# fgnt/pb_chime5

Hardware: AMD Instinct MI355X
Metric: utterance-seconds enhanced/sec/GPU (24ch, 20 EM iters) (higher is better)
Workload: dtype f64

## Files before the change

### pb_chime5_amd/csrc/wpe.hip

```cpp
#include <algorithm>
#include <cmath>
#include <cstdlib>

#include "gss_internal.h"
#include <type_traits>
#include "dense_wave.h"

typedef double v4d __attribute__((ext_vector_type(4)));

namespace {

constexpr int POW_FRAMES = 256;
__global__ __launch_bounds__(POW_FRAMES) void wpe_power_kernel(const cplx *__restrict__ X,
                                                               int64_t T, int D, int psd_context,
                                                               double *__restrict__ raw,
                                                               double *__restrict__ w) {
    extern __shared__ __attribute__((aligned(16))) char smem[];
    double *ps = reinterpret_cast<double *>(smem);
    __shared__ double red[POW_FRAMES / 64];
    const int f = blockIdx.x, tid = threadIdx.x;
    const cplx *Xf = X + (int64_t)f * T * D;
    double *wout = w + (int64_t)f * T;
    double *wf = psd_context > 0 ? raw + (int64_t)f * T : wout;
    const int DP = D + 1;
// ... 553 lines not shown
    if (threadIdx.x == 0 && blockIdx.x < 8192) {
        g_corr_trace[blockIdx.x * 6 + 0] = xcd;
        g_corr_trace[blockIdx.x * 6 + 1] = wall_clock64();
        g_corr_trace[blockIdx.x * 6 + 2] = clock64();
    }
#endif
    int live = 0;
    if (threadIdx.x == 0) {
        ring[0] = corr_fetch(counters, F, xcd, live, cq);
        ring[1] = ring[0] < 0 ? -1 : corr_fetch(counters, F, xcd, live, cq);
        ring[2] = -1;
    }
    __syncthreads();

    const uint32_t lane16 = lane * 16;
    auto issue = [&](int fq, int64_t t0, int bq) {
        const __amdgpu_buffer_rsrc_t rsrc_y = __builtin_amdgcn_make_buffer_rsrc(
            const_cast<cplx *>(Y + (int64_t)fq * T * D), 0, (int)(T * D * 16), 0x00020000);
        cplx *Sb = S0 + bq * win;
        const int64_t g0 = (t0 - c) * (int64_t)D;
        if (g0 >= 0 && g0 + win <= T * (int64_t)D) {
            for (int p = wave; p < pieces; p += NW)
                __builtin_amdgcn_raw_ptr_buffer_load_lds(rsrc_y, (lds_void_ptr)(Sb + p * 64), 16,
                                                         lane16, (int)((g0 + p * 64) * 16), 0, 0);
        } else {
            for (int p = wave; p < pieces; p += NW) {
                const int64_t gp = g0 + p * 64;
                const uint32_t voff = (uint32_t)((gp + lane) * 16);
                if (gp >= 0) {
                    __builtin_amdgcn_raw_ptr_buffer_load_lds(rsrc_y, (lds_void_ptr)(Sb + p * 64),
                                                             16, voff, 0, 0, 0);
                } else if (gp + lane < 0) {
                    Sb[p * 64 + lane] = c_make(0.0, 0.0);
                } else {
                    __builtin_amdgcn_raw_ptr_buffer_load_lds(rsrc_y, (lds_void_ptr)(Sb + p * 64),
                                                             16, voff, 0, 0, 0);
                }
            }
        }
        if (wave == NW - 1 && lane < CORR_KT / 2) {
            const __amdgpu_buffer_rsrc_t rsrc_w = __builtin_amdgcn_make_buffer_rsrc(
                const_cast<double *>(w + (int64_t)fq * T), 0, (int)(T * 8), 0x00020000);
            __builtin_amdgcn_raw_ptr_buffer_load_lds(rsrc_w, (lds_void_ptr)(w0 + bq * CORR_KT), 16,
                                                     lane16, (int)(t0 * 8), 0, 0);
        }
    };

    int item = __builtin_amdgcn_readfirstlane(ring[0]);
    if (item < 0) return;
    int b = 0;
    issue(item >> 12, 0, 0);
    __syncthreads();
    for (int k = 0; item >= 0; ++k) {
        const int next = __builtin_amdgcn_readfirstlane(ring[(k + 1) % 3]);
        int fetched = -1;
        if (threadIdx.x == 0 && next >= 0) fetched = corr_fetch(counters, F, xcd, live, cq);
        const int f = item >> 12, grp = item & 4095;
        const int tile_id = grp * NW + wave;
        const bool active = tile_id < ntiles;
        const CorrTile tl = tiles[active ? tile_id : 0];
        const int mask = __builtin_amdgcn_readfirstlane(active ? tl.mask : 1);
        int *ring_slot = &ring[(k + 2) % 3];
#define CORR_CASE(M)                                                                              \
    case M:                                                                                       \
        corr_item_dma<M, NW, BLOCKED>(T, D, n, c, win, S0, w0, tl, active, f, next < 0 ? -1 : next >> 12, \
                                 b, issue, ring_slot, fetched, R, P);                             \
        break
#define CORR_CASE_RG(RG)                                                                          \
    case 15 + 16 * RG:                                                                            \
        if constexpr (!BLOCKED)                                                                   \
            corr_item_dma<15 + 16 * RG, NW, false>(T, D, n, c, win, S0, w0, tl, active, f,        \
                                                   next < 0 ? -1 : next >> 12, b, issue,          \
                                                   ring_slot, fetched, R, P);                     \
        break
        switch (BLOCKED ? mask & 15 : mask) {
            CORR_CASE(1);
            CORR_CASE(3);
            CORR_CASE(5);
            CORR_CASE(11);
            CORR_CASE_RG(1);
            CORR_CASE_RG(2);
            CORR_CASE_RG(3);
            default:
                corr_item_dma<15, NW, BLOCKED>(T, D, n, c, win, S0, w0, tl, active, f,
                                          next < 0 ? -1 : next >> 12, b, issue, ring_slot, fetched,
                                          R, P);
        }
#undef CORR_CASE
#undef CORR_CASE_RG
        item = next;
#ifdef GSS_CORR_TRACE
        if (threadIdx.x == 0 && blockIdx.x < 8192) {
            g_corr_trace[blockIdx.x * 6 + 3] = wall_clock64();
            g_corr_trace[blockIdx.x * 6 + 4] = clock64();
            g_corr_trace[blockIdx.x * 6 + 5] = k + 1;
        }
#endif
    }
}

#ifndef GSS_UPD_PREFETCH
#define GSS_UPD_PREFETCH 1
#endif
constexpr int CH_NB = 48;
constexpr int UD_LD = CH_NB + 1;

constexpr size_t DIAG_LDS = sizeof(cplx) * 2 * UD_LD + sizeof(double) * CH_NB;

__device__ inline void chol_diag_block(cplx *A, int n, int j0, cplx *Ud, double *dinv,
                                       int32_t *zero_pivots) {
    const int tid = threadIdx.x, tx = tid & 15, ty = tid >> 4;
    const int nb = min(CH_NB, n - j0);
    cplx reg[3][3];
#pragma unroll
    for (int a = 0; a < 3; ++a)
#pragma unroll
        for (int b = 0; b < 3; ++b) {
            const int i = ty + 16 * a, k = tx + 16 * b;
            reg[a][b] = (k >= i && k < nb) ? A[(int64_t)(j0 + i) * n + j0 + k] : c_make(0.0, 0.0);
        }
    if (!chol_inverse_sweep<16, 3, false, true>(reg, nb, Ud, UD_LD, dinv, tx, ty)) {
        if (tid < nb && dinv[tid] == 0.0) atomicAdd(zero_pivots, 1);
    }
#pragma unroll
    for (int a = 0; a < 3; ++a) {
        const int i = ty + 16 * a;
        const double di = i < nb ? dinv[i] : 0.0;
#pragma unroll
        for (int b = 0; b < 3; ++b) {
            const int k = tx + 16 * b;
            if (b < a || i >= nb || k >= nb) continue;
            const cplx raw = reg[a][b];
            A[(int64_t)(j0 + i) * n + j0 + k] =
                k == i ? c_make(di > 0.0 ? sqrt(raw.x) : 0.0, 0.0) : c_scale(raw, di);
        }
    }
}

__global__ __launch_bounds__(256) void chol_diag_kernel(cplx *__restrict__ R, int n, int j0,
                                                        int32_t *__restrict__ zero_pivots) {
    __shared__ __attribute__((aligned(16))) char smem[DIAG_LDS];
    cplx *Ud = reinterpret_cast<cplx *>(smem);
    double *dinv = reinterpret_cast<double *>(Ud + 2 * UD_LD);
    chol_diag_block(R + (int64_t)blockIdx.x * n * n, n, j0, Ud, dinv, zero_pivots);
}

constexpr int UDP_SIZE = 16 * (CH_NB + 1) + 16 * (CH_NB - 16 + 1) + 16 * (CH_NB - 32 + 1);
__device__ __forceinline__ int udp_off(int row, int col) {
    const int b = row >> 4;
    const int base = b == 0 ? 0 : b == 1 ? 16 * (CH_NB + 1) : 16 * (CH_NB + 1) + 16 * (CH_NB - 16 + 1);
    return base + (row & 15) * (CH_NB - 16 * b + 1) + col - 16 * b;
}

__device__ inline void chol_panel_tile(cplx *A, cplx *Z, int n, int D, int j0, int nb, int ct,
                                       const cplx *Ud, const double *dinv, int lane) {
    const int ntrail = n - j0 - nb;
    const int li = lane & 15, lk = lane >> 4;
    const int nct_a = (ntrail + 15) / 16;
    cplx *base;
    int64_t stride;
    int ncols;
    if (ct < nct_a) {
        base = A + (int64_t)j0 * n + j0 + nb + 16 * ct;
        stride = n;
        ncols = min(16, ntrail - 16 * ct);
    } else {
        base = Z + (int64_t)j0 * D + 16 * (ct - nct_a);
        stride = D;
        ncols = min(16, D - 16 * (ct - nct_a));
    }
    cplx bv[CH_NB / 4];
#pragma unroll
    for (int ks = 0; ks < CH_NB / 4; ++ks) {
        const int row = 4 * ks + lk;
        bv[ks] = (row < nb && li < ncols) ? base[row * stride + li] : c_make(0.0, 0.0);
    }
    v4d xre[3], xim[3];
#pragma unroll
    for (int it = 0; it < 3; ++it) {
        v4d tre, tim;
#pragma unroll
        for (int r = 0; r < 4; ++r) {
            tre[r] = bv[4 * it + r].x;
            tim[r] = bv[4 * it + r].y;
        }
        const int i = 16 * it + li;
#pragma unroll
        for (int jt = 0; jt < it; ++jt)
#pragma unroll
            for (int ks = 0; ks < 4; ++ks) {
                const int k = 16 * jt + 4 * ks + lk;
                const cplx u = Ud[udp_off(k, i)];
                tre = __builtin_amdgcn_mfma_f64_16x16x4f64(-u.x, xre[jt][ks], tre, 0, 0, 0);
                tim = __builtin_amdgcn_mfma_f64_16x16x4f64(-u.x, xim[jt][ks], tim, 0, 0, 0);
                tre = __builtin_amdgcn_mfma_f64_16x16x4f64(-u.y, xim[jt][ks], tre, 0, 0, 0);
                tim = __builtin_amdgcn_mfma_f64_16x16x4f64(u.y, xre[jt][ks], tim, 0, 0, 0);
            }
        xre[it] = (v4d){0.0, 0.0, 0.0, 0.0};
        xim[it] = (v4d){0.0, 0.0, 0.0, 0.0};
#pragma unroll
        for (int ks = 0; ks < 4; ++ks) {
            const int k = 16 * it + 4 * ks + lk;
            cplx w = Ud[udp_off(i, k)];
            if (k == i) w = c_make(i < nb ? dinv[i] : 0.0, 0.0);
            if (k > i) w = c_make(0.0, 0.0);
            xre[it] = __builtin_amdgcn_mfma_f64_16x16x4f64(w.x, tre[ks], xre[it], 0, 0, 0);
            xim[it] = __builtin_amdgcn_mfma_f64_16x16x4f64(w.x, tim[ks], xim[it], 0, 0, 0);
            xre[it] = __builtin_amdgcn_mfma_f64_16x16x4f64(-w.y, tim[ks], xre[it], 0, 0, 0);
            xim[it] = __builtin_amdgcn_mfma_f64_16x16x4f64(w.y, tre[ks], xim[it], 0, 0, 0);
        }
    }
#pragma unroll
    for (int it = 0; it < 3; ++it)
#pragma unroll
        for (int r = 0; r < 4; ++r) {
            const int row = 16 * it + lk + 4 * r;
            if (row < nb && li < ncols) base[row * stride + li] = c_make(xre[it][r], xim[it][r]);
        }
}

__device__ inline void chol_stage_diag(const cplx *A, int n, int j0, int nb, cplx *Ud, double *dinv) {
    const int tid = threadIdx.x;
    constexpr int WL = CH_NB * CH_NB / 256;
    static_assert(WL * 256 == CH_NB * CH_NB, "block size");
    cplx wv[WL];
#pragma unroll
    for (int s = 0; s < WL; ++s) {
        const int idx = tid + 256 * s;
        const int i = idx / CH_NB, k = idx - i * CH_NB;
        wv[s] = c_make(0.0, 0.0);
        if (i < nb && k < nb && k >= (i & ~15)) wv[s] = A[(int64_t)(j0 + i) * n + j0 + k];
    }
#pragma unroll
    for (int s = 0; s < WL; ++s) {
        const int idx = tid + 256 * s;
        const int i = idx / CH_NB, k = idx - i * CH_NB;
        if (k >= (i & ~15)) Ud[udp_off(i, k)] = wv[s];
        if (k == i) dinv[i] = wv[s].x > 0.0 ? 1.0 / wv[s].x : 0.0;
    }
}

__global__ __launch_bounds__(256) void chol_trsm_kernel(cplx *__restrict__ R,
                                                        cplx *__restrict__ P, int F, int n,
                                                        int D, int j0) {
    extern __shared__ __attribute__((aligned(16))) char smem[];
    cplx *Ud = reinterpret_cast<cplx *>(smem);
    double *dinv = reinterpret_cast<double *>(Ud + UDP_SIZE);
    const int tid = threadIdx.x;
    const int nb = min(CH_NB, n - j0);
    const int ntrail = n - j0 - nb;
    const int npanel = (ntrail + 15) / 16 + (D + 15) / 16;
    int f, grp;
    if (!xcd_group_map((npanel + 3) / 4, F, f, grp)) return;
    cplx *A = R + (int64_t)f * n * n;
    cplx *Z = P + (int64_t)f * n * D;
    chol_stage_diag(A, n, j0, nb, Ud, dinv);
    __syncthreads();
    const int ct = grp * 4 + (tid >> 6);
    if (ct < npanel) chol_panel_tile(A, Z, n, D, j0, nb, ct, Ud, dinv, tid & 63);
}

struct UpdTile {
    int row_off, col_off, is_p, pad;
};

template <int TM, int TN, bool PREFETCH>
__device__ inline void chol_update_tile(cplx *A, cplx *Z, int n, int D, int j0, int nb,
                                        const UpdTile tl, int lane) {
    const int li = lane & 15, lk = lane >> 4;
    const cplx *panel = A + (int64_t)j0 * n;
    const cplx *zpanel = Z + (int64_t)j0 * D;
    const int ncols = tl.is_p ? D : n;

    auto load_ops = [&](int ks, cplx (&a)[TM], cplx (&b)[TN]) {
        const int kk = 4 * ks + lk;
        const bool kv = kk < nb;
#pragma unroll
        for (int m = 0; m < TM; ++m) {
            const int ri = tl.row_off + 16 * m + li;
            a[m] = (kv && ri < n) ? panel[(int64_t)kk * n + ri] : c_make(0.0, 0.0);
        }
#pragma unroll
        for (int m = 0; m < TN; ++m) {
            const int ci = tl.col_off + 16 * m + li;
            b[m] = c_make(0.0, 0.0);
            if (kv && ci < ncols)
                b[m] = tl.is_p ? zpanel[(int64_t)kk * D + ci] : panel[(int64_t)kk * n + ci];
        }
    };

    const int ksteps = (nb + 3) / 4;
    cplx a_cur[TM], b_cur[TN];
    load_ops(0, a_cur, b_cur);

    cplx cv[TM][TN][4];
#pragma unroll
    for (int a = 0; a < TM; ++a)
#pragma unroll
        for (int b = 0; b < TN; ++b)
#pragma unroll
            for (int reg = 0; reg < 4; ++reg) {
                const int r = tl.row_off + 16 * a + lk + 4 * reg;
                const int c = tl.col_off + 16 * b + li;
                cv[a][b][reg] = c_make(0.0, 0.0);
                if (r < n && c < ncols) cv[a][b][reg] = tl.is_p ? Z[(int64_t)r * D + c] : A[(int64_t)r * n + c];
            }
    v4d t1[TM][TN], t2[TM][TN], t3[TM][TN];
#pragma unroll
    for (int a = 0; a < TM; ++a)
#pragma unroll
        for (int b = 0; b < TN; ++b) {
            t1[a][b] = (v4d){0.0, 0.0, 0.0, 0.0};
            t2[a][b] = (v4d){0.0, 0.0, 0.0, 0.0};
            t3[a][b] = (v4d){0.0, 0.0, 0.0, 0.0};
        }
    constexpr int PD = GSS_UPD_PREFETCH;
    cplx a_ring[PD][TM], b_ring[PD][TN];
#pragma unroll
    for (int p = 0; p < PD; ++p)
        if (PREFETCH && p + 1 < ksteps) load_ops(p + 1, a_ring[p], b_ring[p]);
    for (int ks = 0; ks < ksteps; ++ks) {
        cplx a_new[TM], b_new[TN];
        if (PREFETCH) {
            if (ks + PD + 1 < ksteps) load_ops(ks + PD + 1, a_new, b_new);
        } else if (ks > 0) {
            load_ops(ks, a_cur, b_cur);
        }
        double as[TM], bd[TN];
#pragma unroll
        for (int m = 0; m < TM; ++m) as[m] = a_cur[m].x + a_cur[m].y;
#pragma unroll
        for (int m = 0; m < TN; ++m) bd[m] = b_cur[m].x - b_cur[m].y;
#pragma unroll
        for (int a = 0; a < TM; ++a)
#pragma unroll
            for (int b = 0; b < TN; ++b) {
                t1[a][b] = __builtin_amdgcn_mfma_f64_16x16x4f64(a_cur[a].x, b_cur[b].x, t1[a][b], 0, 0, 0);
                t2[a][b] = __builtin_amdgcn_mfma_f64_16x16x4f64(a_cur[a].y, b_cur[b].y, t2[a][b], 0, 0, 0);
                t3[a][b] = __builtin_amdgcn_mfma_f64_16x16x4f64(as[a], bd[b], t3[a][b], 0, 0, 0);
            }
        if (PREFETCH) {
#pragma unroll
            for (int m = 0; m < TM; ++m) {
                a_cur[m] = a_ring[0][m];
#pragma unroll
                for (int p = 0; p + 1 < PD; ++p) a_ring[p][m] = a_ring[p + 1][m];
                a_ring[PD - 1][m] = a_new[m];
            }
#pragma unroll
            for (int m = 0; m < TN; ++m) {
                b_cur[m] = b_ring[0][m];
#pragma unroll
                for (int p = 0; p + 1 < PD; ++p) b_ring[p][m] = b_ring[p + 1][m];
                b_ring[PD - 1][m] = b_new[m];
            }
        }
    }
#pragma unroll
    for (int a = 0; a < TM; ++a)
#pragma unroll
        for (int b = 0; b < TN; ++b)
#pragma unroll
            for (int reg = 0; reg < 4; ++reg) {
                const int r = tl.row_off + 16 * a + lk + 4 * reg;
                const int c = tl.col_off + 16 * b + li;
                if (r < n && c < ncols) {
                    const cplx v = c_make(cv[a][b][reg].x - (t1[a][b][reg] + t2[a][b][reg]),
                                          cv[a][b][reg].y - ((t1[a][b][reg] - t2[a][b][reg]) - t3[a][b][reg]));
                    if (tl.is_p) Z[(int64_t)r * D + c] = v;
                    else A[(int64_t)r * n + c] = v;
                }
            }
}

constexpr int UPD_WAVES = 4;

template <int TM, int TN, bool PREFETCH>
__global__ __launch_bounds__(64 * UPD_WAVES) void chol_update_kernel(cplx *__restrict__ R,
                                                          cplx *__restrict__ P, int F, int n,
                                                          int D, int j0, int nb,
                                                          const UpdTile *__restrict__ tiles,
                                                          int ntiles, int ndiag, int j0_next,
                                                          int32_t *__restrict__ zero_pivots) {
    __shared__ __attribute__((aligned(16))) char smem[DIAG_LDS];
    const int F8 = ndiag > 0 ? (F + 7) / 8 * 8 : 0;
    const bool diag_group = (int)blockIdx.x < F8;
    int f, grp;
    if (diag_group) {
        f = blockIdx.x;
        grp = 0;
        if (f >= F) return;
    } else {
        const int L = blockIdx.x - F8, nsub = (ntiles - ndiag + UPD_WAVES - 1) / UPD_WAVES;
        const int sg = L / (8 * nsub), rem = L - sg * 8 * nsub;
        grp = rem >> 3;
        f = sg * 8 + (rem & 7);
        if (f >= F) return;
    }
    const int wave = __builtin_amdgcn_readfirstlane(threadIdx.x >> 6), lane = threadIdx.x & 63;
    cplx *A = R + (int64_t)f * n * n, *Z = P + (int64_t)f * n * D;
    if (diag_group) {
        __builtin_amdgcn_s_setprio(3);
        for (int t = wave; t < ndiag; t += UPD_WAVES)
            chol_update_tile<TM, TN, PREFETCH>(A, Z, n, D, j0, nb, tiles[t], lane);
        __syncthreads();
        if (wave >= 4) return;
        cplx *Ud = reinterpret_cast<cplx *>(smem);
        double *dinv = reinterpret_cast<double *>(Ud + 2 * UD_LD);
        chol_diag_block(A, n, j0_next, Ud, dinv, zero_pivots);
        return;
    }
    const int tile_id = ndiag + grp * UPD_WAVES + wave;
    if (tile_id >= ntiles) return;
    chol_update_tile<TM, TN, PREFETCH>(A, Z, n, D, j0, nb, tiles[tile_id], lane);
}

constexpr int BS_LD = 33;
constexpr int BS_OPS = 6 * 4 * 64;

__device__ inline void chol_backsolve_body(const cplx *A, cplx *Z, int n, int D, cplx *S,
                                           cplx *OP) {
    const int wave = __builtin_amdgcn_readfirstlane(threadIdx.x >> 6), lane = threadIdx.x & 63;
    const int li = lane & 15, lk = lane >> 4;
    const int nblk = (n + CH_NB - 1) / CH_NB;
    const int a = wave;
    for (int c0 = 0; c0 < D; c0 += 32) {
        for (int J = nblk - 1; J >= 0; --J) {
            const int j0 = J * CH_NB, nb = min(CH_NB, n - j0);
            if (a == 3) {
                const cplx *Ad = A + (int64_t)j0 * n + j0;
                auto fetch = [&](int row, int col) {
                    const bool ok = row < nb && col < nb;
                    const cplx v = Ad[(int64_t)(ok ? row : 0) * n + (ok ? col : 0)];
                    return c_make(ok ? v.x : 0.0, ok ? v.y : 0.0);
                };
                cplx wop[3][4], uop[3][4];
                double dg[3];
#pragma unroll
                for (int it = 0; it < 3; ++it) {
#pragma unroll
                    for (int ks = 0; ks < 4; ++ks) wop[it][ks] = fetch(16 * it + 4 * ks + lk, 16 * it + li);
                    dg[it] = fetch(16 * it + li, 16 * it + li).x;
                }
#pragma unroll
                for (int ks = 0; ks < 4; ++ks) {
                    uop[0][ks] = fetch(16 + li, 32 + 4 * ks + lk);
                    uop[1][ks] = fetch(li, 16 + 4 * ks + lk);
                    uop[2][ks] = fetch(li, 32 + 4 * ks + lk);
                }
#pragma unroll
                for (int it = 0; it < 3; ++it) {
                    const double ndinv = dg[it] > 0.0 ? -1.0 / dg[it] : 0.0;
#pragma unroll
                    for (int ks = 0; ks < 4; ++ks) {
                        const int k = 4 * ks + lk;
                        const cplx w = wop[it][ks];
                        OP[(it * 4 + ks) * 64 + lane] =
                            c_make(k == li ? ndinv : (k < li ? 0.0 : -w.x), k <= li ? 0.0 : -w.y);
                        OP[((3 + it) * 4 + ks) * 64 + lane] = uop[it][ks];
                    }
                }
            } else {
                v4d acc_re[2], acc_im[2];
#pragma unroll
                for (int b = 0; b < 2; ++b)
#pragma unroll
                    for (int reg = 0; reg < 4; ++reg) {
                        const int rl = 16 * a + lk + 4 * reg, col = c0 + 16 * b + li;
                        cplx v = c_make(0.0, 0.0);
                        if (rl < nb && col < D) v = Z[(int64_t)(j0 + rl) * D + col];
                        acc_re[b][reg] = v.x;
                        acc_im[b][reg] = v.y;
                    }
                const int kbeg = j0 + nb;
                const int ksteps = (n - kbeg + 3) / 4;
                const int arow = 16 * a + li;
                auto load_ops = [&](int ks, cplx &u, cplx (&g)[2]) {
                    const int kk = kbeg + 4 * ks + lk;
                    const bool kv = kk < n;
                    u = (kv && arow < nb) ? A[(int64_t)(j0 + arow) * n + kk] : c_make(0.0, 0.0);
#pragma unroll
                    for (int b = 0; b < 2; ++b) {
                        const int col = c0 + 16 * b + li;
                        g[b] = (kv && col < D) ? Z[(int64_t)kk * D + col] : c_make(0.0, 0.0);
                    }
                };
                constexpr int PD = 6;
                cplx u_r[PD], g_r[PD][2];
#pragma unroll
                for (int p = 0; p < PD; ++p) load_ops(p, u_r[p], g_r[p]);
                for (int ks0 = 0; ks0 < ksteps; ks0 += PD) {
#pragma unroll
                    for (int p = 0; p < PD; ++p) {
                        const double nur = -u_r[p].x, nui = -u_r[p].y, ui = u_r[p].y;
                        const double g0r = g_r[p][0].x, g0i = g_r[p][0].y;
                        const double g1r = g_r[p][1].x, g1i = g_r[p][1].y;
                        load_ops(ks0 + p + PD, u_r[p], g_r[p]);
                        __builtin_amdgcn_sched_barrier(0);
                        acc_re[0] = __builtin_amdgcn_mfma_f64_16x16x4f64(nur, g0r, acc_re[0], 0, 0, 0);
                        acc_im[0] = __builtin_amdgcn_mfma_f64_16x16x4f64(nur, g0i, acc_im[0], 0, 0, 0);
                        acc_re[1] = __builtin_amdgcn_mfma_f64_16x16x4f64(nur, g1r, acc_re[1], 0, 0, 0);
                        acc_im[1] = __builtin_amdgcn_mfma_f64_16x16x4f64(nur, g1i, acc_im[1], 0, 0, 0);
                        acc_re[0] = __builtin_amdgcn_mfma_f64_16x16x4f64(ui, g0i, acc_re[0], 0, 0, 0);
                        acc_im[0] = __builtin_amdgcn_mfma_f64_16x16x4f64(nui, g0r, acc_im[0], 0, 0, 0);
                        acc_re[1] = __builtin_amdgcn_mfma_f64_16x16x4f64(ui, g1i, acc_re[1], 0, 0, 0);
                        acc_im[1] = __builtin_amdgcn_mfma_f64_16x16x4f64(nui, g1r, acc_im[1], 0, 0, 0);
                        __builtin_amdgcn_sched_barrier(0);
                    }
                }
#pragma unroll
                for (int b = 0; b < 2; ++b)
#pragma unroll
                    for (int reg = 0; reg < 4; ++reg)
                        S[(16 * a + lk + 4 * reg) * BS_LD + 16 * b + li] =
                            c_make(acc_re[b][reg], acc_im[b][reg]);
            }
            __syncthreads();
            const int b = 3 - a;
            if (a >= 2 && c0 + 16 * b < D) {
                v4d xre[3], xim[3], nxim[3];
#pragma unroll
                for (int st = 0; st < 3; ++st) {
                    const int it = 2 - st;
                    v4d tre, tim;
#pragma unroll
                    for (int reg = 0; reg < 4; ++reg) {
                        const cplx sv = S[(16 * it + lk + 4 * reg) * BS_LD + 16 * b + li];
                        tre[reg] = -sv.x;
                        tim[reg] = -sv.y;
                    }
#pragma unroll
                    for (int sj = 0; sj < st; ++sj)
#pragma unroll
                        for (int ks = 0; ks < 4; ++ks) {
                            const int jt = 2 - sj;
                            const cplx u = OP[((3 + (it == 1 ? 0 : jt)) * 4 + ks) * 64 + lane];
                            tre = __builtin_amdgcn_mfma_f64_16x16x4f64(u.x, xre[jt][ks], tre, 0, 0, 0);
                            tim = __builtin_amdgcn_mfma_f64_16x16x4f64(u.x, xim[jt][ks], tim, 0, 0, 0);
                            tre = __builtin_amdgcn_mfma_f64_16x16x4f64(u.y, nxim[jt][ks], tre, 0, 0, 0);
                            tim = __builtin_amdgcn_mfma_f64_16x16x4f64(u.y, xre[jt][ks], tim, 0, 0, 0);
                        }
                    const v4d ntre = -tre;
                    xre[it] = (v4d){0.0, 0.0, 0.0, 0.0};
                    xim[it] = (v4d){0.0, 0.0, 0.0, 0.0};
#pragma unroll
                    for (int ks = 0; ks < 4; ++ks) {
                        const cplx pw = OP[(it * 4 + ks) * 64 + lane];
                        xre[it] = __builtin_amdgcn_mfma_f64_16x16x4f64(pw.x, tre[ks], xre[it], 0, 0, 0);
                        xim[it] = __builtin_amdgcn_mfma_f64_16x16x4f64(pw.x, tim[ks], xim[it], 0, 0, 0);
                        xre[it] = __builtin_amdgcn_mfma_f64_16x16x4f64(pw.y, tim[ks], xre[it], 0, 0, 0);
                        xim[it] = __builtin_amdgcn_mfma_f64_16x16x4f64(pw.y, ntre[ks], xim[it], 0, 0, 0);
                    }
                    nxim[it] = -xim[it];
#pragma unroll
                    for (int reg = 0; reg < 4; ++reg) {
                        const int rl = 16 * it + lk + 4 * reg, col = c0 + 16 * b + li;
                        if (rl < nb && col < D)
                            Z[(int64_t)(j0 + rl) * D + col] = c_make(xre[it][reg], xim[it][reg]);
                    }
                }
            }
            __syncthreads();
        }
    }
}

__global__ __launch_bounds__(256, 3) void chol_backsolve_kernel(const cplx *__restrict__ R,
                                                             cplx *__restrict__ P, int n, int D) {
    __shared__ cplx S[CH_NB * BS_LD];
    __shared__ cplx OP[BS_OPS];
    const int f = blockIdx.x;
    chol_backsolve_body(R + (int64_t)f * n * n, P + (int64_t)f * n * D, n, D, S, OP);
}

template <int TA, int NB, int NWV, int WRAPS, bool TAIL, int RG>
__device__ __forceinline__ void wpe_apply_body(const cplx *__restrict__ Y,
                                               const cplx *__restrict__ G, int F, int64_t T, int D,
                                               int n, int c, cplx *__restrict__ X) {
    constexpr int WAVE_FRAMES = 16 * TA, WG_FRAMES = NWV * WAVE_FRAMES;
    extern __shared__ __attribute__((aligned(16))) char smem[];
    cplx *S = reinterpret_cast<cplx *>(smem);
    const int DP = D | 1;
    int f, chunk;
    if (!xcd_group_map((int)((T + WG_FRAMES - 1) / WG_FRAMES), F, f, chunk)) return;
    const int64_t t0 = (int64_t)chunk * WG_FRAMES;
    const cplx *Yf = Y + (int64_t)f * T * D;
    const cplx *Gf = G + (int64_t)f * n * D;
    const int frames_lds = WG_FRAMES + c + 2;
    const int64_t fr0 = t0 - c;
    constexpr int PRE = 14, NT = 64 * NWV;
    const int total = frames_lds * D;
    for (int base = 0; base < total; base += NT * PRE) {
        cplx v[PRE];
#pragma unroll
        for (int j = 0; j < PRE; ++j) {
            const int idx = base + (int)threadIdx.x + NT * j;
            const int64_t fr = fr0 + idx / D;
            v[j] = c_make(0.0, 0.0);
            if (idx < total && fr >= 0 && fr < T) v[j] = Yf[fr0 * D + idx];
        }
#pragma unroll
        for (int j = 0; j < PRE; ++j) {
            const int idx = base + (int)threadIdx.x + NT * j;
            const int fl = idx / D, d = idx - fl * D;
            if (idx < total) S[fl * DP + d] = v[j];
        }
    }
    __syncthreads();
    const int wave = threadIdx.x >> 6, lane = threadIdx.x & 63;
    const int li = lane & 15, lk = lane >> 4;
    const int wf0 = wave * WAVE_FRAMES;
    if (t0 + wf0 >= T) return;
    static_assert(RG == 0 || NB == 2, "remainder groups replace the second of two channel tiles");
    constexpr int NBL = RG > 0 ? 1 : NB;
    constexpr int NG = RG > 0 ? RG : 1;
    v4d acc_re[TA][NBL], acc_im[TA][NBL], acc_t2[TA][NBL];
    double sml_re[TA][NG], sml_im[TA][NG], sml_t2[TA][NG];
#pragma unroll
    for (int a = 0; a < TA; ++a) {
#pragma unroll
        for (int b = 0; b < NBL; ++b) {
            acc_re[a][b] = (v4d){0.0, 0.0, 0.0, 0.0};
            acc_im[a][b] = (v4d){0.0, 0.0, 0.0, 0.0};
            acc_t2[a][b] = (v4d){0.0, 0.0, 0.0, 0.0};
        }
#pragma unroll
        for (int g = 0; g < NG; ++g) sml_re[a][g] = sml_im[a][g] = sml_t2[a][g] = 0.0;
    }
    const int ksteps = (n + 3) / 4;
    const int lds_last = frames_lds * DP - 1;
    constexpr int NBG = NBL + RG;
    int goff[NBG], goff_max[NBG];
#pragma unroll
    for (int b = 0; b < NBG; ++b) {
        const int col = min(b < NBL ? 16 * b + li : 16 + 4 * (b - NBL) + (lane & 3), D - 1);
        goff[b] = min(lk, n - 1) * D + col;
        goff_max[b] = (n - 1) * D + col;
    }
    auto load_g = [&](int, cplx (&g)[NBG]) {
#pragma unroll
        for (int b = 0; b < NBG; ++b) {
            g[b] = Gf[goff[b]];
            goff[b] = min(goff[b] + 4 * D, goff_max[b]);
        }
    };
    int rm = lk % D, lin = (lk / D) * DP + rm;
    int ubase[TA];
#pragma unroll
    for (int a = 0; a < TA; ++a) ubase[a] = (wf0 + 16 * a + li) * DP;
    auto load_u = [&](cplx (&u)[TA]) {
#pragma unroll
        for (int a = 0; a < TA; ++a) u[a] = S[min(ubase[a] + lin, lds_last)];
        rm += 4;
        lin += 4;
#pragma unroll
        for (int w = 0; w < WRAPS; ++w) {
            const bool wrap = rm >= D;
            rm -= wrap ? D : 0;
            lin += wrap ? DP - D : 0;
        }
    };
    auto step = [&](int ks, const cplx (&g)[NBG], const cplx (&u)[TA]) {
        const bool ok = !TAIL || 4 * ks + lk < n;
        double ur[TA], ui[TA], gr[NBG], gi[NBG];
#pragma unroll
        for (int a = 0; a < TA; ++a) {
            ur[a] = ok ? u[a].x : 0.0;
            ui[a] = ok ? u[a].y : 0.0;
        }
#pragma unroll
        for (int b = 0; b < NBG; ++b) {
            gr[b] = g[b].x;
            gi[b] = g[b].y;
        }
        double us[TA], gd[NBG];
#pragma unroll
        for (int a = 0; a < TA; ++a) us[a] = ur[a] + ui[a];
#pragma unroll
        for (int b = 0; b < NBG; ++b) gd[b] = gr[b] - gi[b];
#pragma unroll
        for (int a = 0; a < TA; ++a) {
#pragma unroll
            for (int b = 0; b < NBL; ++b) {
                acc_re[a][b] = __builtin_amdgcn_mfma_f64_16x16x4f64(ur[a], gr[b], acc_re[a][b], 0, 0, 0);
                acc_t2[a][b] = __builtin_amdgcn_mfma_f64_16x16x4f64(ui[a], gi[b], acc_t2[a][b], 0, 0, 0);
                acc_im[a][b] = __builtin_amdgcn_mfma_f64_16x16x4f64(us[a], gd[b], acc_im[a][b], 0, 0, 0);
            }
#pragma unroll
            for (int g = 0; g < RG; ++g) {
                const int b = NBL + g;
                sml_re[a][g] = __builtin_amdgcn_mfma_f64_4x4x4f64(ur[a], gr[b], sml_re[a][g], 0, 0, 0);
                sml_t2[a][g] = __builtin_amdgcn_mfma_f64_4x4x4f64(ui[a], gi[b], sml_t2[a][g], 0, 0, 0);
                sml_im[a][g] = __builtin_amdgcn_mfma_f64_4x4x4f64(us[a], gd[b], sml_im[a][g], 0, 0, 0);
            }
        }
    };
    cplx g0[NBG], g1[NBG], u0[TA], u1[TA];
    load_g(0, g0);
    load_u(u0);
    for (int ks = 0; ks < ksteps; ks += 2) {
        load_g(ks + 1, g1);
        load_u(u1);
        __builtin_amdgcn_sched_barrier(0);
        step(ks, g0, u0);
        __builtin_amdgcn_sched_barrier(0);
        load_g(ks + 2, g0);
        load_u(u0);
        __builtin_amdgcn_sched_barrier(0);
        step(ks + 1, g1, u1);
        __builtin_amdgcn_sched_barrier(0);
    }
#pragma unroll
    for (int a = 0; a < TA; ++a)
#pragma unroll
        for (int b = 0; b < NBL; ++b)
#pragma unroll
            for (int reg = 0; reg < 4; ++reg) {
                const int fl = wf0 + 16 * a + lk + 4 * reg;
                const int d = 16 * b + li;
                const int64_t t = t0 + fl;
                if (d < D && t < T) {
                    const cplx y = S[(fl + c) * DP + d];
                    const double pre = acc_re[a][b][reg] + acc_t2[a][b][reg];
                    const double pim = (acc_im[a][b][reg] - acc_re[a][b][reg]) + acc_t2[a][b][reg];
                    X[((int64_t)f * T + t) * D + d] = c_make(y.x - pre, y.y - pim);
// ... 585 lines not shown
        double best = (double)((D + 15) / 16) * n;
        for (int ph = 2; ph <= 4; ++ph) {
            if (ph_env > 0 && ph != ph_env) continue;
            const int nt = (ph * D + 15) / 16;
            if (nt > 3 || D < 2) continue;
            const double cost = (double)nt * (n + (ph - 1) * D) / ph;
            const int fl = 64 * ph + c + 2;
            const size_t lds = sizeof(cplx) * ((size_t)fl * (D | 1) + fl / ph + 1 + (size_t)(n + 1) * (D | 1));
            if (lds > (ph_env == ph ? 160 : 64) * 1024) continue;
            if (cost < 0.75 * best || ph_env == ph) {
                ph_env_taken = ph_env_taken || ph_env == ph;
                best = cost;
                apply_ph = ph;
                apply_nt = nt;
                packed_lds = lds;
            }
        }
        if (ph_env == 1) apply_ph = 1;
        if (!ph_env_taken) {
            static bool warned = false;
            if (!warned)
                fprintf(stderr, "libgss_hip: GSS_VARIANT apply_ph=%d is not available for D=%d taps=%d "
                                "(column tiles or LDS); using the default\n", ph_env, D, taps);
            warned = true;
        }
    }
    using apply_packed_t = void (*)(const cplx *, const cplx *, int, int64_t, int, int, int, cplx *);
    apply_packed_t packed_fn = nullptr;
    const bool apply_gglobal = apply_ph == 1 && D > 16 && 2 * D <= 48 && D % 4 == 0 && n % 4 == 0 &&
                               gss_variant_set("apply_gglobal") && gss_variant("apply_ph", 0) == 0 &&
                               !gss_variant_set("apply_generic");
    if (apply_gglobal) {
        apply_ph = 2;
        apply_nt = 3;
        const int fl = 64 * 2 + c + 2;
        packed_lds = sizeof(cplx) * ((size_t)fl * (D | 1) + fl / 2 + 1);
        packed_fn = wpe_apply_packed_kernel<2, 3, false>;
    } else
    if (apply_ph > 1) {
        static const apply_packed_t table[3][3] = {
            {wpe_apply_packed_kernel<2, 1>, wpe_apply_packed_kernel<2, 2>, wpe_apply_packed_kernel<2, 3>},
            {wpe_apply_packed_kernel<3, 1>, wpe_apply_packed_kernel<3, 2>, wpe_apply_packed_kernel<3, 3>},
            {wpe_apply_packed_kernel<4, 1>, wpe_apply_packed_kernel<4, 2>, wpe_apply_packed_kernel<4, 3>}};
        packed_fn = table[apply_ph - 2][apply_nt - 1];
        static const apply_packed_t table_small[3][3] = {
            {wpe_apply_packed_kernel<2, 1, true, 4, 1>, wpe_apply_packed_kernel<2, 2, true, 4, 1>, wpe_apply_packed_kernel<2, 3, true, 4, 1>},
            {wpe_apply_packed_kernel<3, 1, true, 4, 1>, wpe_apply_packed_kernel<3, 2, true, 4, 1>, wpe_apply_packed_kernel<3, 3, true, 4, 1>},
            {wpe_apply_packed_kernel<4, 1, true, 4, 1>, wpe_apply_packed_kernel<4, 2, true, 4, 1>, wpe_apply_packed_kernel<4, 3, true, 4, 1>}};
        if ((64 * apply_ph + c + 2) * D <= 4 * 256 && n * D <= 256 && !gss_variant_set("apply_generic"))
            packed_fn = table_small[apply_ph - 2][apply_nt - 1];
        if (packed_lds > 64 * 1024)
            GSS_HIP_CHECK(ctx, hipFuncSetAttribute(reinterpret_cast<const void *>(packed_fn),
                                                   hipFuncAttributeMaxDynamicSharedMemorySize,
                                                   (int)packed_lds));
    }
    GSS_REQUIRE(ctx, corr_lds <= 160 * 1024 && apply_lds <= 160 * 1024, GSS_ERR_UNSUPPORTED,
                "wpe: taps=%d D=%d needs more LDS than a CU has", taps, D);
    if (apply_lds > 64 * 1024)
        GSS_HIP_CHECK(ctx, hipFuncSetAttribute(reinterpret_cast<const void *>(apply_fn),
                                               hipFuncAttributeMaxDynamicSharedMemorySize,
                                               (int)apply_lds));
    if (corr_lds > 64 * 1024)
        GSS_HIP_CHECK(ctx, hipFuncSetAttribute(reinterpret_cast<const void *>(corr_fn),
                                               hipFuncAttributeMaxDynamicSharedMemorySize,
                                               (int)corr_lds));
    const int corr_pieces = (int)(((size_t)(CORR_KT + c + padf) * D + 63) / 64);
    const size_t corr_dma_lds = 2 * (sizeof(cplx) * 64 * (size_t)corr_pieces + sizeof(double) * CORR_KT);
    const bool corr_persist = corr_ts == 2 && (int64_t)T * D * 16 < (1LL << 31) &&
                              corr_dma_lds <= 80 * 1024;
    if (corr_persist && !nw_forced) corr_nw = 4;
    const bool corr_blocked = corr_persist && gss_variant_set("corr_blocked");
    auto corr_persist_fn = corr_blocked ? (corr_nw == 2 ? wpe_corr_persist_kernel<2, true>
                                                        : wpe_corr_persist_kernel<4, true>)
                                        : (corr_nw == 2 ? wpe_corr_persist_kernel<2>
                                                        : wpe_corr_persist_kernel<4>);
    CorrQueue corr_queue{(ntiles + corr_nw - 1) / corr_nw, 0};
    int corr_slots = 0;
    if (corr_persist) {
        for (int g = 0; g < corr_queue.ngroups; ++g)
            if (corr_tile_cost(tiles[g * corr_nw]) >= 12) corr_queue.gh = g + 1;
        if (corr_dma_lds > 64 * 1024)
            GSS_HIP_CHECK(ctx, hipFuncSetAttribute(reinterpret_cast<const void *>(corr_persist_fn),
                                                   hipFuncAttributeMaxDynamicSharedMemorySize,
                                                   (int)corr_dma_lds));
        int per_cu = 0, cus = 0;
        GSS_HIP_CHECK(ctx, hipOccupancyMaxActiveBlocksPerMultiprocessor(
                               &per_cu, reinterpret_cast<const void *>(corr_persist_fn), 64 * corr_nw,
                               corr_dma_lds));
        GSS_HIP_CHECK(ctx, hipDeviceGetAttribute(&cus, hipDeviceAttributeMultiprocessorCount, ctx->device));
        corr_slots = std::min(std::max(per_cu, 1) * cus, corr_queue.ngroups * F);
    }

    for (int it = 0; it < iterations; ++it) {
        const cplx *cur = it == 0 ? Y : X;
        if (!cw) {
            GSS_PROF(ctx, "wpe_power");
            GSS_TRY(wpe_power_launch(ctx, cur, F, T, D, psd_context, raw, w_own));
        }
        if (corr_persist) {
            GSS_HIP_CHECK(ctx, hipMemsetAsync(corr_counters, 0, 8 * 16 * sizeof(int), ctx->stream));
            GSS_PROF(ctx, "wpe_corr");
            hipLaunchKernelGGL(corr_persist_fn, dim3(corr_slots), dim3(64 * corr_nw), corr_dma_lds,
                               ctx->stream, Y, w, F, T, D, n, c, corr_pieces, tiles_dev, ntiles,
                               corr_queue, corr_counters, R, P);
            GSS_LAUNCH_CHECK(ctx, "wpe_corr_persist_kernel");
        } else {
            GSS_PROF(ctx, "wpe_corr");
            if (ksplit_fn)
                hipLaunchKernelGGL(ksplit_fn, dim3(xcd_grid(ntiles, F)), dim3(64 * corr_ks), corr_lds,
                                   ctx->stream, Y, w, F, T, D, n, c, padf, tiles_dev, ntiles, R, P);
            else
                hipLaunchKernelGGL(corr_fn, dim3(xcd_grid((ntiles + corr_nw - 1) / corr_nw, F)),
                                   dim3(64 * corr_nw), corr_lds,
                                   ctx->stream, Y, w, F, T, D, n, c, padf, tiles_dev, ntiles, R, P);
            GSS_LAUNCH_CHECK(ctx, "wpe_corr_kernel");
        }
        {
            const int nblk = (n + CH_NB - 1) / CH_NB;
            const bool detail = gss_variant_set("prof_detail");
            static const char *trsm_names[] = {"wpe_chol_trsm_J0", "wpe_chol_trsm_J1", "wpe_chol_trsm_J2",
                                               "wpe_chol_trsm_J3", "wpe_chol_trsm_J4", "wpe_chol_trsm_J5+"};
            static const char *upd_names[] = {"wpe_chol_update_J0", "wpe_chol_update_J1", "wpe_chol_update_J2",
                                              "wpe_chol_update_J3", "wpe_chol_update_J4", "wpe_chol_update_J5+"};
            for (int J = 0; J < nblk; ++J) {
                const int j0 = J * CH_NB, nb = std::min(CH_NB, n - j0);
                if (J == 0 || upd_ndiag[J - 1] == 0) {
                    GSS_PROF(ctx, "wpe_chol_diag");
                    hipLaunchKernelGGL(chol_diag_kernel, dim3(F), dim3(256), 0, ctx->stream, R, n, j0,
                                       zero_pivots);
                    GSS_LAUNCH_CHECK(ctx, "chol_diag_kernel");
                }
                {
                    GSS_PROF(ctx, detail ? trsm_names[std::min(J, 5)] : "wpe_chol_trsm");
                    const int npanel = (n - j0 - nb + 15) / 16 + (D + 15) / 16;
                    hipLaunchKernelGGL(chol_trsm_kernel, dim3(xcd_grid((npanel + 3) / 4, F)),
                                       dim3(256), panel_lds, ctx->stream, R, P, F, n, D, j0);
                    GSS_LAUNCH_CHECK(ctx, "chol_trsm_kernel");
                }
                const int nupd = upd_count[J];
                if (nupd > 0) {
                    GSS_PROF(ctx, detail ? upd_names[std::min(J, 5)] : "wpe_chol_update");
                    const int ndiag = upd_ndiag[J];
                    const dim3 g((ndiag > 0 ? (F + 7) / 8 * 8 : 0) +
                                 xcd_grid((nupd - ndiag + UPD_WAVES - 1) / UPD_WAVES, F)), b(64 * UPD_WAVES);
                    const UpdTile *tl = upd_dev + upd_start[J];
                    hipLaunchKernelGGL((chol_update_kernel<1, 1, true>), g, b, 0, ctx->stream, R, P, F, n, D, upd_j0[J],
                                       std::min(upd_k[J], n - upd_j0[J]), tl, nupd, ndiag,
                                       (J + 1) * CH_NB, zero_pivots);
                    GSS_LAUNCH_CHECK(ctx, "chol_update_kernel");
                }
            }
            {
                GSS_PROF(ctx, "wpe_backsolve");
                hipLaunchKernelGGL(chol_backsolve_kernel, dim3(F), dim3(256), 0, ctx->stream, R, P, n,
                                   D);
                GSS_LAUNCH_CHECK(ctx, "chol_backsolve_kernel");
            }
        }
        {
            GSS_PROF(ctx, "wpe_apply");
            if (packed_fn) {
                const int wg_frames = 64 * apply_ph;
                hipLaunchKernelGGL(packed_fn, dim3(xcd_grid((int)((T + wg_frames - 1) / wg_frames), F)),
                                   dim3(256), packed_lds, ctx->stream, Y, P, F, T, D, n, c, X);
            } else {
                hipLaunchKernelGGL(apply_fn,
                                   dim3(xcd_grid((int)((T + apply_frames - 1) / apply_frames), F)),
                                   dim3(64 * apply_nwv), apply_lds, ctx->stream, Y, P, F, T, D, n, c, X);
            }
            GSS_LAUNCH_CHECK(ctx, "wpe_apply_kernel");
        }
    }
    if (part < 0)
        GSS_HIP_CHECK(ctx, hipMemcpyAsync(ctx->status_host + (cw ? cw->status_word : 2), zero_pivots,
                                          sizeof(int32_t), hipMemcpyDeviceToHost, ctx->stream));
    return GSS_OK;
}


int wpe_copy_zero_pivots(gss_ctx *ctx) {
    if (!ctx->wpe_tiles) return GSS_OK;
    const int32_t *zero_pivots =
        reinterpret_cast<const int32_t *>(reinterpret_cast<const CorrTile *>(ctx->wpe_tiles) + 1024 + 4096);
    GSS_HIP_CHECK(ctx, hipMemcpyAsync(ctx->status_host + 2, zero_pivots, sizeof(int32_t),
                                      hipMemcpyDeviceToHost, ctx->stream));
    return GSS_OK;
}

int selftest_mfma_run(gss_ctx *ctx) {
    double *out = nullptr;
    GSS_HIP_CHECK(ctx, hipMalloc(reinterpret_cast<void **>(&out), sizeof(double) * 320));
    hipLaunchKernelGGL(mfma_selftest_kernel, dim3(1), dim3(64), 0, ctx->stream, out);
    double host[320];
    hipError_t e = hipMemcpyAsync(host, out, sizeof(host), hipMemcpyDeviceToHost, ctx->stream);
    if (e == hipSuccess) e = hipStreamSynchronize(ctx->stream);
    (void)hipFree(out);
    if (e != hipSuccess) return gss_fail(ctx, GSS_ERR_HIP, "mfma selftest: %s", hipGetErrorString(e));
    for (int i = 0; i < 16; ++i)
        for (int j = 0; j < 16; ++j) {
            const double want = (double)(i + 1) * 100.0 * (double)(j + 1);
            if (host[i * 16 + j] != want)
                return gss_fail(ctx, GSS_ERR_UNSUPPORTED,
                                "f64 MFMA fragment layout mismatch at (%d,%d): got %g want %g", i,
                                j, host[i * 16 + j], want);
        }
    for (int q = 0; q < 4; ++q)
        for (int i = 0; i < 4; ++i)
            for (int j = 0; j < 4; ++j) {
                double want = 0.0;
                for (int k = 0; k < 4; ++k)
                    want += (double)(1 + i + 4 * q + 16 * k) * 100.0 * (double)(1 + j + 4 * q + 16 * k);
                const double got = host[256 + j + 4 * q + 16 * i];
                if (got != want)
                    return gss_fail(ctx, GSS_ERR_UNSUPPORTED,
                                    "f64 4x4x4 MFMA fragment layout mismatch at block %d (%d,%d): got %g want %g",
                                    q, i, j, got, want);
            }
    return GSS_OK;
}
```

Before: 1110.

## Split Cholesky backsolve across 16-column tiles and prefetch trsm panel loads

The backsolve kernel now launches one workgroup per (frequency, 16-column tile) instead of one per frequency looping over 32-column chunks. This spreads work across more CUs, shrinks LDS use (packed triangular W operand, smaller S buffer) and raises the occupancy hint. The trsm kernel now issues the first part of its panel loads before staging the diagonal block, so global loads overlap with the LDS staging and barrier. The trade-off is that each column tile reloads the diagonal and U operands and redoes that setup, and two MFMA accumulators per wave become one.

```diff
diff --git a/pb_chime5_amd/csrc/wpe.hip b/pb_chime5_amd/csrc/wpe.hip
--- a/pb_chime5_amd/csrc/wpe.hip
+++ b/pb_chime5_amd/csrc/wpe.hip
@@ -729,29 +729,34 @@
     return base + (row & 15) * (CH_NB - 16 * b + 1) + col - 16 * b;
 }
 
-__device__ inline void chol_panel_tile(cplx *A, cplx *Z, int n, int D, int j0, int nb, int ct,
+struct PanelTile {
+    cplx *base;
+    int stride, ncols;
+};
+
+__device__ inline PanelTile chol_panel_where(cplx *A, cplx *Z, int n, int D, int j0, int nb,
+                                             int ct) {
+    const int ntrail = n - j0 - nb;
+    const int nct_a = (ntrail + 15) / 16;
+    if (ct < nct_a) return {A + (int64_t)j0 * n + j0 + nb + 16 * ct, n, min(16, ntrail - 16 * ct)};
+    return {Z + (int64_t)j0 * D + 16 * (ct - nct_a), D, max(0, min(16, D - 16 * (ct - nct_a)))};
+}
+
+template <int KS0, int KS1>
+__device__ inline void chol_panel_load(const PanelTile t, int nb, int lane, cplx (&bv)[CH_NB / 4]) {
+    const int li = lane & 15, lk = lane >> 4;
+#pragma unroll
+    for (int ks = KS0; ks < KS1; ++ks) {
+        const int row = 4 * ks + lk;
+        bv[ks] = (row < nb && li < t.ncols) ? t.base[row * t.stride + li] : c_make(0.0, 0.0);
+    }
+}
+
+__device__ inline void chol_panel_tile(const PanelTile t, int nb, const cplx (&bv)[CH_NB / 4],
                                        const cplx *Ud, const double *dinv, int lane) {
-    const int ntrail = n - j0 - nb;
     const int li = lane & 15, lk = lane >> 4;
-    const int nct_a = (ntrail + 15) / 16;
-    cplx *base;
-    int64_t stride;
-    int ncols;
-    if (ct < nct_a) {
-        base = A + (int64_t)j0 * n + j0 + nb + 16 * ct;
-        stride = n;
-        ncols = min(16, ntrail - 16 * ct);
-    } else {
-        base = Z + (int64_t)j0 * D + 16 * (ct - nct_a);
-        stride = D;
-        ncols = min(16, D - 16 * (ct - nct_a));
-    }
-    cplx bv[CH_NB / 4];
-#pragma unroll
-    for (int ks = 0; ks < CH_NB / 4; ++ks) {
-        const int row = 4 * ks + lk;
-        bv[ks] = (row < nb && li < ncols) ? base[row * stride + li] : c_make(0.0, 0.0);
-    }
+    cplx *base = t.base;
+    const int stride = t.stride, ncols = t.ncols;
     v4d xre[3], xim[3];
 #pragma unroll
     for (int it = 0; it < 3; ++it) {
@@ -817,7 +822,7 @@
     }
 }
 
-__global__ __launch_bounds__(256) void chol_trsm_kernel(cplx *__restrict__ R,
+__global__ __launch_bounds__(256, 5) void chol_trsm_kernel(cplx *__restrict__ R,
                                                         cplx *__restrict__ P, int F, int n,
                                                         int D, int j0) {
     extern __shared__ __attribute__((aligned(16))) char smem[];
@@ -831,10 +836,14 @@
     if (!xcd_group_map((npanel + 3) / 4, F, f, grp)) return;
     cplx *A = R + (int64_t)f * n * n;
     cplx *Z = P + (int64_t)f * n * D;
+    const int ct = grp * 4 + (tid >> 6);
+    const PanelTile tile = chol_panel_where(A, Z, n, D, j0, nb, ct);
+    cplx bv[CH_NB / 4];
+    chol_panel_load<0, 4>(tile, nb, tid & 63, bv);
     chol_stage_diag(A, n, j0, nb, Ud, dinv);
     __syncthreads();
-    const int ct = grp * 4 + (tid >> 6);
-    if (ct < npanel) chol_panel_tile(A, Z, n, D, j0, nb, ct, Ud, dinv, tid & 63);
+    chol_panel_load<4, CH_NB / 4>(tile, nb, tid & 63, bv);
+    if (ct < npanel) chol_panel_tile(tile, nb, bv, Ud, dinv, tid & 63);
 }
 
 struct UpdTile {
@@ -992,162 +1001,157 @@
     chol_update_tile<TM, TN, PREFETCH>(A, Z, n, D, j0, nb, tiles[tile_id], lane);
 }
 
-constexpr int BS_LD = 33;
-constexpr int BS_OPS = 6 * 4 * 64;
-
-__device__ inline void chol_backsolve_body(const cplx *A, cplx *Z, int n, int D, cplx *S,
-                                           cplx *OP) {
+constexpr int BS_S = 3 * 4 * 64;
+constexpr int BS_W = 3 * 136;
+constexpr int BS_U = 3 * 4 * 64;
+
+__device__ inline void chol_backsolve_body(const cplx *A, cplx *Z, int n, int D, int c0,
+                                           cplx *S, cplx *OPW, cplx *OPU) {
     const int wave = __builtin_amdgcn_readfirstlane(threadIdx.x >> 6), lane = threadIdx.x & 63;
     const int li = lane & 15, lk = lane >> 4;
     const int nblk = (n + CH_NB - 1) / CH_NB;
     const int a = wave;
-    for (int c0 = 0; c0 < D; c0 += 32) {
-        for (int J = nblk - 1; J >= 0; --J) {
-            const int j0 = J * CH_NB, nb = min(CH_NB, n - j0);
-            if (a == 3) {
-                const cplx *Ad = A + (int64_t)j0 * n + j0;
-                auto fetch = [&](int row, int col) {
-                    const bool ok = row < nb && col < nb;
-                    const cplx v = Ad[(int64_t)(ok ? row : 0) * n + (ok ? col : 0)];
-                    return c_make(ok ? v.x : 0.0, ok ? v.y : 0.0);
-                };
-                cplx wop[3][4], uop[3][4];
-                double dg[3];
-#pragma unroll
-                for (int it = 0; it < 3; ++it) {
-#pragma unroll
-                    for (int ks = 0; ks < 4; ++ks) wop[it][ks] = fetch(16 * it + 4 * ks + lk, 16 * it + li);
-                    dg[it] = fetch(16 * it + li, 16 * it + li).x;
+    for (int J = nblk - 1; J >= 0; --J) {
+        const int j0 = J * CH_NB, nb = min(CH_NB, n - j0);
+        if (a == 3) {
+            const cplx *Ad = A + (int64_t)j0 * n + j0;
+            auto fetch = [&](int row, int col) {
+                const bool ok = row < nb && col < nb;
+                const cplx v = Ad[(int64_t)(ok ? row : 0) * n + (ok ? col : 0)];
+                return c_make(ok ? v.x : 0.0, ok ? v.y : 0.0);
+            };
+            cplx wop[3][4];
+            double dg[3];
+#pragma unroll
+            for (int it = 0; it < 3; ++it) {
+#pragma unroll
+                for (int ks = 0; ks < 4; ++ks) wop[it][ks] = fetch(16 * it + 4 * ks + lk, 16 * it + li);
+                dg[it] = fetch(16 * it + li, 16 * it + li).x;
+            }
+#pragma unroll
+            for (int it = 0; it < 3; ++it) {
+                const double ndinv = dg[it] > 0.0 ? -1.0 / dg[it] : 0.0;
+#pragma unroll
+                for (int ks = 0; ks < 4; ++ks) {
+                    const int k = 4 * ks + lk;
+                    const cplx w = wop[it][ks];
+                    if (k >= li)
+                        OPW[it * 136 + k * (k + 1) / 2 + li] =
+                            c_make(k == li ? ndinv : -w.x, k == li ? 0.0 : -w.y);
                 }
+            }
+            cplx uop[3][4];
+#pragma unroll
+            for (int ks = 0; ks < 4; ++ks) {
+                uop[0][ks] = fetch(16 + li, 32 + 4 * ks + lk);
+                uop[1][ks] = fetch(li, 16 + 4 * ks + lk);
+                uop[2][ks] = fetch(li, 32 + 4 * ks + lk);
+            }
+#pragma unroll
+            for (int it = 0; it < 3; ++it)
+#pragma unroll
+                for (int ks = 0; ks < 4; ++ks) OPU[(it * 4 + ks) * 64 + lane] = uop[it][ks];
+        } else {
+            v4d acc_re, acc_im;
+            const int col = c0 + li;
+#pragma unroll
+            for (int reg = 0; reg < 4; ++reg) {
+                const int rl = 16 * a + lk + 4 * reg;
+                cplx v = c_make(0.0, 0.0);
+                if (rl < nb && col < D) v = Z[(int64_t)(j0 + rl) * D + col];
+                acc_re[reg] = v.x;
+                acc_im[reg] = v.y;
+            }
+            const int kbeg = j0 + nb;
+            const int ksteps = (n - kbeg + 3) / 4;
+            const int arow = 16 * a + li;
+            auto load_ops = [&](int ks, cplx &u, cplx &g) {
+                const int kk = kbeg + 4 * ks + lk;
+                const bool kv = kk < n;
+                u = (kv && arow < nb) ? A[(int64_t)(j0 + arow) * n + kk] : c_make(0.0, 0.0);
+                g = (kv && col < D) ? Z[(int64_t)kk * D + col] : c_make(0.0, 0.0);
+            };
+            constexpr int PD = 6;
+            cplx u_r[PD], g_r[PD];
+#pragma unroll
+            for (int p = 0; p < PD; ++p) load_ops(p, u_r[p], g_r[p]);
+            for (int ks0 = 0; ks0 < ksteps; ks0 += PD) {
+#pragma unroll
+                for (int p = 0; p < PD; ++p) {
+                    const double nur = -u_r[p].x, nui = -u_r[p].y, ui = u_r[p].y;
+                    const double gr = g_r[p].x, gi = g_r[p].y;
+                    load_ops(ks0 + p + PD, u_r[p], g_r[p]);
+                    __builtin_amdgcn_sched_barrier(0);
+                    acc_re = __builtin_amdgcn_mfma_f64_16x16x4f64(nur, gr, acc_re, 0, 0, 0);
+                    acc_im = __builtin_amdgcn_mfma_f64_16x16x4f64(nur, gi, acc_im, 0, 0, 0);
+                    acc_re = __builtin_amdgcn_mfma_f64_16x16x4f64(ui, gi, acc_re, 0, 0, 0);
+                    acc_im = __builtin_amdgcn_mfma_f64_16x16x4f64(nui, gr, acc_im, 0, 0, 0);
+                    __builtin_amdgcn_sched_barrier(0);
+                }
+            }
+#pragma unroll
+            for (int reg = 0; reg < 4; ++reg)
+                S[(a * 4 + reg) * 64 + lane] = c_make(acc_re[reg], acc_im[reg]);
+        }
+        __syncthreads();
+        if (a == 3) {
+            v4d xre[3], xim[3];
+#pragma unroll
+            for (int st = 0; st < 3; ++st) {
+                const int it = 2 - st;
+                v4d tre, tim;
+#pragma unroll
+                for (int reg = 0; reg < 4; ++reg) {
+                    const cplx sv = S[(it * 4 + reg) * 64 + lane];
+                    tre[reg] = -sv.x;
+                    tim[reg] = -sv.y;
+                }
+#pragma unroll
+                for (int sj = 0; sj < st; ++sj)
+#pragma unroll
+                    for (int ks = 0; ks < 4; ++ks) {
+                        const int jt = 2 - sj;
+                        const cplx u = OPU[((it == 1 ? 0 : jt) * 4 + ks) * 64 + lane];
+                        tre = __builtin_amdgcn_mfma_f64_16x16x4f64(u.x, xre[jt][ks], tre, 0, 0, 0);
+                        tim = __builtin_amdgcn_mfma_f64_16x16x4f64(u.x, xim[jt][ks], tim, 0, 0, 0);
+                        tre = __builtin_amdgcn_mfma_f64_16x16x4f64(-u.y, xim[jt][ks], tre, 0, 0, 0);
+                        tim = __builtin_amdgcn_mfma_f64_16x16x4f64(u.y, xre[jt][ks], tim, 0, 0, 0);
+                    }
+                const v4d ntre = -tre;
+                xre[it] = (v4d){0.0, 0.0, 0.0, 0.0};
+                xim[it] = (v4d){0.0, 0.0, 0.0, 0.0};
 #pragma unroll
                 for (int ks = 0; ks < 4; ++ks) {
-                    uop[0][ks] = fetch(16 + li, 32 + 4 * ks + lk);
-                    uop[1][ks] = fetch(li, 16 + 4 * ks + lk);
-                    uop[2][ks] = fetch(li, 32 + 4 * ks + lk);
+                    const int k = 4 * ks + lk;
+                    cplx pw = c_make(0.0, 0.0);
+                    if (k >= li) pw = OPW[it * 136 + k * (k + 1) / 2 + li];
+                    xre[it] = __builtin_amdgcn_mfma_f64_16x16x4f64(pw.x, tre[ks], xre[it], 0, 0, 0);
+                    xim[it] = __builtin_amdgcn_mfma_f64_16x16x4f64(pw.x, tim[ks], xim[it], 0, 0, 0);
+                    xre[it] = __builtin_amdgcn_mfma_f64_16x16x4f64(pw.y, tim[ks], xre[it], 0, 0, 0);
+                    xim[it] = __builtin_amdgcn_mfma_f64_16x16x4f64(pw.y, ntre[ks], xim[it], 0, 0, 0);
                 }
 #pragma unroll
-                for (int it = 0; it < 3; ++it) {
-                    const double ndinv = dg[it] > 0.0 ? -1.0 / dg[it] : 0.0;
-#pragma unroll
-                    for (int ks = 0; ks < 4; ++ks) {
-                        const int k = 4 * ks + lk;
-                        const cplx w = wop[it][ks];
-                        OP[(it * 4 + ks) * 64 + lane] =
-                            c_make(k == li ? ndinv : (k < li ? 0.0 : -w.x), k <= li ? 0.0 : -w.y);
-                        OP[((3 + it) * 4 + ks) * 64 + lane] = uop[it][ks];
-                    }
+                for (int reg = 0; reg < 4; ++reg) {
+                    const int rl = 16 * it + lk + 4 * reg, col = c0 + li;
+                    if (rl < nb && col < D)
+                        Z[(int64_t)(j0 + rl) * D + col] = c_make(xre[it][reg], xim[it][reg]);
                 }
-            } else {
-                v4d acc_re[2], acc_im[2];
-#pragma unroll
-                for (int b = 0; b < 2; ++b)
-#pragma unroll
-                    for (int reg = 0; reg < 4; ++reg) {
-                        const int rl = 16 * a + lk + 4 * reg, col = c0 + 16 * b + li;
-                        cplx v = c_make(0.0, 0.0);
-                        if (rl < nb && col < D) v = Z[(int64_t)(j0 + rl) * D + col];
-                        acc_re[b][reg] = v.x;
-                        acc_im[b][reg] = v.y;
-                    }
-                const int kbeg = j0 + nb;
-                const int ksteps = (n - kbeg + 3) / 4;
-                const int arow = 16 * a + li;
-                auto load_ops = [&](int ks, cplx &u, cplx (&g)[2]) {
-                    const int kk = kbeg + 4 * ks + lk;
-                    const bool kv = kk < n;
-                    u = (kv && arow < nb) ? A[(int64_t)(j0 + arow) * n + kk] : c_make(0.0, 0.0);
-#pragma unroll
-                    for (int b = 0; b < 2; ++b) {
-                        const int col = c0 + 16 * b + li;
-                        g[b] = (kv && col < D) ? Z[(int64_t)kk * D + col] : c_make(0.0, 0.0);
-                    }
-                };
-                constexpr int PD = 6;
-                cplx u_r[PD], g_r[PD][2];
-#pragma unroll
-                for (int p = 0; p < PD; ++p) load_ops(p, u_r[p], g_r[p]);
-                for (int ks0 = 0; ks0 < ksteps; ks0 += PD) {
-#pragma unroll
-                    for (int p = 0; p < PD; ++p) {
-                        const double nur = -u_r[p].x, nui = -u_r[p].y, ui = u_r[p].y;
-                        const double g0r = g_r[p][0].x, g0i = g_r[p][0].y;
-                        const double g1r = g_r[p][1].x, g1i = g_r[p][1].y;
-                        load_ops(ks0 + p + PD, u_r[p], g_r[p]);
-                        __builtin_amdgcn_sched_barrier(0);
-                        acc_re[0] = __builtin_amdgcn_mfma_f64_16x16x4f64(nur, g0r, acc_re[0], 0, 0, 0);
-                        acc_im[0] = __builtin_amdgcn_mfma_f64_16x16x4f64(nur, g0i, acc_im[0], 0, 0, 0);
-                        acc_re[1] = __builtin_amdgcn_mfma_f64_16x16x4f64(nur, g1r, acc_re[1], 0, 0, 0);
-                        acc_im[1] = __builtin_amdgcn_mfma_f64_16x16x4f64(nur, g1i, acc_im[1], 0, 0, 0);
-                        acc_re[0] = __builtin_amdgcn_mfma_f64_16x16x4f64(ui, g0i, acc_re[0], 0, 0, 0);
-                        acc_im[0] = __builtin_amdgcn_mfma_f64_16x16x4f64(nui, g0r, acc_im[0], 0, 0, 0);
-                        acc_re[1] = __builtin_amdgcn_mfma_f64_16x16x4f64(ui, g1i, acc_re[1], 0, 0, 0);
-                        acc_im[1] = __builtin_amdgcn_mfma_f64_16x16x4f64(nui, g1r, acc_im[1], 0, 0, 0);
-                        __builtin_amdgcn_sched_barrier(0);
-                    }
-                }
-#pragma unroll
-                for (int b = 0; b < 2; ++b)
-#pragma unroll
-                    for (int reg = 0; reg < 4; ++reg)
-                        S[(16 * a + lk + 4 * reg) * BS_LD + 16 * b + li] =
-                            c_make(acc_re[b][reg], acc_im[b][reg]);
-            }
-            __syncthreads();
-            const int b = 3 - a;
-            if (a >= 2 && c0 + 16 * b < D) {
-                v4d xre[3], xim[3], nxim[3];
-#pragma unroll
-                for (int st = 0; st < 3; ++st) {
-                    const int it = 2 - st;
-                    v4d tre, tim;
-#pragma unroll
-                    for (int reg = 0; reg < 4; ++reg) {
-                        const cplx sv = S[(16 * it + lk + 4 * reg) * BS_LD + 16 * b + li];
-                        tre[reg] = -sv.x;
-                        tim[reg] = -sv.y;
-                    }
-#pragma unroll
-                    for (int sj = 0; sj < st; ++sj)
-#pragma unroll
-                        for (int ks = 0; ks < 4; ++ks) {
-                            const int jt = 2 - sj;
-                            const cplx u = OP[((3 + (it == 1 ? 0 : jt)) * 4 + ks) * 64 + lane];
-                            tre = __builtin_amdgcn_mfma_f64_16x16x4f64(u.x, xre[jt][ks], tre, 0, 0, 0);
-                            tim = __builtin_amdgcn_mfma_f64_16x16x4f64(u.x, xim[jt][ks], tim, 0, 0, 0);
-                            tre = __builtin_amdgcn_mfma_f64_16x16x4f64(u.y, nxim[jt][ks], tre, 0, 0, 0);
-                            tim = __builtin_amdgcn_mfma_f64_16x16x4f64(u.y, xre[jt][ks], tim, 0, 0, 0);
-                        }
-                    const v4d ntre = -tre;
-                    xre[it] = (v4d){0.0, 0.0, 0.0, 0.0};
-                    xim[it] = (v4d){0.0, 0.0, 0.0, 0.0};
-#pragma unroll
-                    for (int ks = 0; ks < 4; ++ks) {
-                        const cplx pw = OP[(it * 4 + ks) * 64 + lane];
-                        xre[it] = __builtin_amdgcn_mfma_f64_16x16x4f64(pw.x, tre[ks], xre[it], 0, 0, 0);
-                        xim[it] = __builtin_amdgcn_mfma_f64_16x16x4f64(pw.x, tim[ks], xim[it], 0, 0, 0);
-                        xre[it] = __builtin_amdgcn_mfma_f64_16x16x4f64(pw.y, tim[ks], xre[it], 0, 0, 0);
-                        xim[it] = __builtin_amdgcn_mfma_f64_16x16x4f64(pw.y, ntre[ks], xim[it], 0, 0, 0);
-                    }
-                    nxim[it] = -xim[it];
-#pragma unroll
-                    for (int reg = 0; reg < 4; ++reg) {
-                        const int rl = 16 * it + lk + 4 * reg, col = c0 + 16 * b + li;
-                        if (rl < nb && col < D)
-                            Z[(int64_t)(j0 + rl) * D + col] = c_make(xre[it][reg], xim[it][reg]);
-                    }
-                }
-            }
-            __syncthreads();
-        }
-    }
-}
-
-__global__ __launch_bounds__(256, 3) void chol_backsolve_kernel(const cplx *__restrict__ R,
-                                                             cplx *__restrict__ P, int n, int D) {
-    __shared__ cplx S[CH_NB * BS_LD];
-    __shared__ cplx OP[BS_OPS];
-    const int f = blockIdx.x;
-    chol_backsolve_body(R + (int64_t)f * n * n, P + (int64_t)f * n * D, n, D, S, OP);
+            }
+        }
+        __syncthreads();
+    }
+}
+
+__global__ __launch_bounds__(256, 5) void chol_backsolve_kernel(const cplx *__restrict__ R,
+                                                             cplx *__restrict__ P, int F, int n,
+                                                             int D) {
+    __shared__ cplx S[BS_S];
+    __shared__ cplx OPW[BS_W];
+    __shared__ cplx OPU[BS_U];
+    int f, tile;
+    if (!xcd_group_map((D + 15) / 16, F, f, tile)) return;
+    chol_backsolve_body(R + (int64_t)f * n * n, P + (int64_t)f * n * D, n, D, 16 * tile, S, OPW,
+                        OPU);
 }
 
 template <int TA, int NB, int NWV, int WRAPS, bool TAIL, int RG>
@@ -2039,8 +2043,8 @@
             }
             {
                 GSS_PROF(ctx, "wpe_backsolve");
-                hipLaunchKernelGGL(chol_backsolve_kernel, dim3(F), dim3(256), 0, ctx->stream, R, P, n,
-                                   D);
+                hipLaunchKernelGGL(chol_backsolve_kernel, dim3(xcd_grid((D + 15) / 16, F)), dim3(256),
+                                   0, ctx->stream, R, P, F, n, D);
                 GSS_LAUNCH_CHECK(ctx, "chol_backsolve_kernel");
             }
         }
```

Measured after the change: 1115, median of 6. No clear change (+0.4%).
